# svg-project/Sparse-VideoGen

Hardware: AMD Instinct MI355X
Metric: attn_tflops_svg1_block_sparse (higher is better)
Workload: dtype bf16; 1 GPU; HunyuanVideo T2V hy720p SVG1 sparse layer-call: sample_mse(64 rows) + band attention with fused head placement, cfg=1 H=24 D=128 F=33 P=3600 ctx=256 prompt=64 S=119056 band=15616 density=0.2456; parallelism=single, variant=0, heads=alt

## Files before the change

### include/svg_attn.h

```cpp
#ifndef SVG_ATTN_H_
#define SVG_ATTN_H_

#include <stddef.h>
#include <stdint.h>

#ifdef __cplusplus
extern "C" {
#endif

#define SVG_DTYPE_BF16 0
#define SVG_DTYPE_F16 1
#define SVG_DTYPE_F32 2

#define SVG_OK 0
#define SVG_ERR_BAD_ARG (-1)
#define SVG_ERR_UNSUPPORTED (-2)
#define SVG_ERR_WORKSPACE (-3)
#define SVG_ERR_LAUNCH (-4)

#define SVG_ABI_VERSION 4
int svg_abi_version(void);

const char* svg_strerror(int code);
int svg_last_hip_error(void);
// ... 221 lines not shown
                           void* workspace, size_t workspace_bytes, const int32_t* skip_flag, void* stream);

size_t svg_band_attention_fp8_workspace_bytes(int32_t BH, int32_t S, int32_t D);
int svg_band_attention_fp8(const void* q, const void* k, const void* v, void* o, int32_t BH, int32_t S, int32_t D, int32_t dtype,
                           float sm_scale, const svg_band_mask_t* mask, const svg_perm_desc_t* perm, void* workspace,
                           size_t workspace_bytes, void* stream);
int svg_band_attention_fp8_stage(const void* q, const void* k, const void* v, void* o, int32_t BH, int32_t S, int32_t D, int32_t dtype,
                                 float sm_scale, const svg_band_mask_t* mask, const svg_perm_desc_t* perm, void* workspace,
                                 size_t workspace_bytes, int32_t stage, void* stream);

size_t svg_varblock_attention_fp8_workspace_bytes(int32_t Hq, int32_t Hkv, int32_t QB, int32_t KB, int32_t Sq, int32_t Skv, int32_t D);
int svg_varblock_attention_fp8(const void* q, const void* k, const void* v, void* o, int32_t Hq, int32_t Hkv, int32_t Sq, int32_t Skv,
                               int32_t D, int32_t dtype, float sm_scale, const uint8_t* block_map, const int32_t* q_sizes,
                               const int32_t* k_sizes, int32_t QB, int32_t KB, const int32_t* q_row_idx, const int32_t* kv_row_idx,
                               void* workspace, size_t workspace_bytes, void* stream);

int32_t svg_band_attention_notify_target(int32_t S, const svg_band_mask_t* mask);
int svg_band_attention_notify(const void* q, const void* k, const void* v, void* o, int32_t BH, int32_t S, int32_t D,
                              int32_t dtype, float sm_scale, const svg_band_mask_t* mask, const svg_perm_desc_t* perm,
                              int32_t* done_per_head, int32_t done_words, void* stream);
int svg_wait_counters(const int32_t* counters, int32_t n, int32_t target, void* stream);
int svg_wait_counters_deadline(const int32_t* counters, int32_t n, int32_t target, int32_t timeout_ms, int32_t* timed_out,
                               void* stream);
int32_t svg_band_attention_notify_layout(int32_t S, const svg_band_mask_t* mask, int32_t nseg, int32_t* row_bounds, int32_t* targets);
int svg_band_attention_notify_seg(const void* q, const void* k, const void* v, void* o, int32_t BH, int32_t S, int32_t D,
                                  int32_t dtype, float sm_scale, const svg_band_mask_t* mask, const svg_perm_desc_t* perm,
                                  int32_t* done, int32_t done_words, int32_t nseg, void* stream);
int svg_band_attention_prescaled_notify_seg(const void* q_scaled, const void* k, const void* v, void* o, int32_t BH, int32_t S,
                                            int32_t D, int32_t dtype, const svg_band_mask_t* mask, const svg_perm_desc_t* perm,
                                            int32_t* done, int32_t done_words, int32_t nseg, void* stream);

int32_t svg_band_queue_order(int32_t BH, int32_t S, const svg_band_mask_t* mask, int32_t* out, int32_t out_words);
int svg_debug_band_queue_cap(int32_t max_workgroups);

int svg_debug_pp_trace(uint64_t* out104);

int svg_debug_clock_probe(const int32_t* stop_flag, uint64_t* out2, int32_t max_ms, void* stream);

int svg_debug_wg_trace(uint64_t* out, int32_t n_workgroups);

#ifdef __cplusplus
}
#endif
#endif
```

### sparse-videogen_amd/csrc/attention.hip

```cpp
#include <algorithm>
#include <atomic>
#include <mutex>

#include "attn_core.h"
#include "attn_m16.h"
#include "band_policy.h"

namespace svg {

template <typename T, int D, int NW>
__global__ __launch_bounds__(NW * 64, 2) void band_attn_kernel(typename BandPolicy<T, D, NW>::Params prm) {
    extern __shared__ __attribute__((aligned(16))) char smem[];
    attn_body<T, D, NW, BandPolicy<T, D, NW>>(prm, smem, nullptr);
}

template <typename T, int D>
__global__ __launch_bounds__(512, (D == 64 ? 4 : 2)) void band_attn_pp2_kernel(typename BandPolicy<T, D, 8>::Params prm) {
    extern __shared__ __attribute__((aligned(16))) char smem[];
    attn_body_pp2<T, D, BandPolicy<T, D, 8>, false, 0, false, D == 64>(prm, smem, nullptr);
}
template <typename T>
__global__ __launch_bounds__(512, 4) void band_attn_pp2_switch64_kernel(typename BandPolicy<T, 64, 8>::Params prm,
                                                                        typename BandPolicy<T, 64, 8>::Params prm_alt,
                                                                        const int32_t* __restrict__ flag) {
    extern __shared__ __attribute__((aligned(16))) char smem[];
    if (flag[0] != 0) attn_body_pp2<T, 64, BandPolicy<T, 64, 8>, false, 0, false, true>(prm_alt, smem, nullptr);
    else attn_body_pp2<T, 64, BandPolicy<T, 64, 8>, false, 0, false, true>(prm, smem, nullptr);
}
template <typename T, int D>
__global__ __launch_bounds__(512, 2) void band_attn_pp2q_switch_kernel(typename BandPolicy<T, D, 8>::Params prm,
                                                                       typename BandPolicy<T, D, 8>::Params prm_alt,
                                                                       const int32_t* __restrict__ flag) {
    extern __shared__ __attribute__((aligned(16))) char smem[];
    if (flag[0] != 0) attn_body_pp2<T, D, BandPolicy<T, D, 8>, false, 0, true>(prm_alt, smem, nullptr);
    else attn_body_pp2<T, D, BandPolicy<T, D, 8>, false, 0, true>(prm, smem, nullptr);
}

__global__ __launch_bounds__(512, 2) void band_attn_pp2_frozen_kernel(typename BandPolicy<__bf16, 128, 8>::Params prm) {
    extern __shared__ __attribute__((aligned(16))) char smem[];
    attn_body_pp2<__bf16, 128, BandPolicy<__bf16, 128, 8>, false, 8>(prm, smem, nullptr);
}
template <typename T>
__global__ __launch_bounds__(512, 2) void band_attn_m16_kernel(typename BandPolicy<T, 128, 8>::Params prm) {
    extern __shared__ __attribute__((aligned(16))) char smem[];
    attn_body_m16<T, BandPolicy<T, 128, 8>, false, 1>(prm, smem, nullptr);
}
template <typename T>
__global__ __launch_bounds__(512, 2) void band_attn_m16q_kernel(typename BandPolicy<T, 128, 8>::Params prm) {
    extern __shared__ __attribute__((aligned(16))) char smem[];
    attn_body_m16<T, BandPolicy<T, 128, 8>, false, 1, true>(prm, smem, nullptr);
}
template <typename T, bool PRE = false>
__global__ __launch_bounds__(512, 2) void band_attn_m16_queue_kernel(typename BandPolicy<T, 128, 8>::Params prm, BandQueue qd) {
    extern __shared__ __attribute__((aligned(16))) char smem[];
    using Pol = BandPolicy<T, 128, 8>;
    int* const slot = (int*)(smem + attn_m16_lds_bytes());
    int dry = 0;
    for (;;) {
        if (threadIdx.x == 0) {
            const int xcd = __builtin_amdgcn_s_getreg((31 << 11) | 20) & (kNumXCD - 1);
            int head = -1, qt = 0;
            const int w = qd.take(xcd, dry);
            if (w >= 0) qd.decode(w, head, qt);
            slot[0] = head, slot[1] = qt;
        }
        __syncthreads();
        const int head = __builtin_amdgcn_readfirstlane(slot[0]), qt = __builtin_amdgcn_readfirstlane(slot[1]);
        if (head < 0) break;
        typename Pol::Ctx ctx;
        Pol::init_tile(prm, ctx, head, qt);
        attn_m16_tile<T, Pol, false, 1, PRE>(prm, ctx, smem);
    }
    if (threadIdx.x == 0) qd.leave(gridDim.x);
}
constexpr int kQueueLds = 16;
template <typename T, bool PRE = false>
__global__ __launch_bounds__(512, 2) void band_attn_m16_switch_kernel(typename BandPolicy<T, 128, 8>::Params prm,
                                                                      typename BandPolicy<T, 128, 8>::Params prm_alt,
                                                                      const int32_t* __restrict__ flag) {
    extern __shared__ __attribute__((aligned(16))) char smem[];
    if (flag[0] != 0) attn_body_m16<T, BandPolicy<T, 128, 8>, false, 1, PRE>(prm_alt, smem, nullptr);
    else attn_body_m16<T, BandPolicy<T, 128, 8>, false, 1, PRE>(prm, smem, nullptr);
}
template <typename T, int D>
__global__ __launch_bounds__(512, 2) void band_attn_pp2q_kernel(typename BandPolicy<T, D, 8>::Params prm) {
    extern __shared__ __attribute__((aligned(16))) char smem[];
    attn_body_pp2<T, D, BandPolicy<T, D, 8>, false, 0, true>(prm, smem, nullptr);
}
#ifdef SVG_ABLATIONS
template <typename T, int D, int ABL>
__global__ __launch_bounds__(512, 2) void band_attn_pp2_trace_kernel(typename BandPolicy<T, D, 8>::Params prm) {
    extern __shared__ __attribute__((aligned(16))) char smem[];
    attn_body_pp2<T, D, BandPolicy<T, D, 8>, true, ABL>(prm, smem, nullptr);
}
template <typename T>
__global__ __launch_bounds__(512, 2) void band_attn_m16_trace_kernel(typename BandPolicy<T, 128, 8>::Params prm) {
    extern __shared__ __attribute__((aligned(16))) char smem[];
    attn_body_m16<T, BandPolicy<T, 128, 8>, true>(prm, smem, nullptr);
}
template <typename T, int D>
__global__ __launch_bounds__(512, 2) void band_attn_pp2q_trace_kernel(typename BandPolicy<T, D, 8>::Params prm) {
    extern __shared__ __attribute__((aligned(16))) char smem[];
    attn_body_pp2<T, D, BandPolicy<T, D, 8>, true, 0, true>(prm, smem, nullptr);
}
#endif

int (*g_trace_reader)(uint64_t*, bool, int) = read_trace_here;

enum BandSchedule : int { kBandAuto = 0, kBandLockstep4 = 1, kBandPingPong = 2, kBandW4 = 3, kBandFrozen = 6, kBandM16 = 8 };
static inline int band_default(int D) { return D == 128 ? kBandM16 : kBandPingPong; }

int band_waves_per_tile(int variant) {
    const int v = variant == kBandAuto ? kBandPingPong : variant;
    return v == kBandW4 ? 4 : ((v == kBandPingPong || v == kBandM16) ? 8 : -1);
}
// ... 97 lines not shown
    if ((variant & 0xFF) == 32) {
        opts.trace = true;
        opts.trace_abl = (variant >> 8) & 15;
        return run_band_w4(q, k, v, o, BH, S, D, dtype, sm_scale, mask, perm, opts, st);
    }
    if (variant & 64) {
        trace_abl = (variant >> 8) & 15;
        variant = kBandPingPong;
        g_trace_reader = read_trace_here;
    }
    if (variant == kBandAuto) variant = band_default(D);
    if (opts.done && band_waves_per_tile(variant) < 0) return SVG_ERR_UNSUPPORTED;
    if (opts.strided && variant != kBandM16 && variant != kBandPingPong) return SVG_ERR_UNSUPPORTED;
    if (variant == kBandW4) return run_band_w4(q, k, v, o, BH, S, D, dtype, sm_scale, mask, perm, opts, st);
    if (variant != kBandLockstep4 && variant != kBandPingPong && variant != kBandFrozen && variant != kBandM16) return SVG_ERR_BAD_ARG;
    return dispatch_td(dtype, D, [&](auto t, auto d) -> int {
        using T = decltype(t);
        constexpr int DD = decltype(d)::value;
        using Pol = BandPolicy<T, DD, 8>;
        auto launch = [&](auto kern, int lds) {
            const typename Pol::Params p = make_band_params<Pol, T>(q, k, v, o, BH, S, sm_scale, mask, perm, opts);
            return launch_attn(kern, dim3(p.nqt * BH), 512, lds, st, p);
        };
        auto launch_queue = [&](auto kern_q, auto kern, int lds) {
            const typename Pol::Params p = make_band_params<Pol, T>(q, k, v, o, BH, S, sm_scale, mask, perm, opts);
            int n_cu = 0;
            int32_t* const block = opts.done ? nullptr : band_queue_block(st, n_cu);
            const int cap = band_queue_cap();
            if (!block || (p.nqt * BH <= n_cu && cap == 0)) return launch_attn(kern, dim3(p.nqt * BH), 512, lds, st, p);
            BandQueue qd = make_band_queue<Pol>(p);
            qd.ctr = block;
            int n_wg = std::min(qd.n_items, n_cu);
            if (cap > 0) n_wg = std::min(n_wg, cap);
            return launch_attn(kern_q, dim3(n_wg), 512, lds + kQueueLds, st, p, qd);
        };
        auto launch_switch = [&](auto kern, int lds) {
            const typename Pol::Params a = make_band_params<Pol, T>(q, k, v, o, BH, S, sm_scale, mask, perm, opts);
            const typename Pol::Params b = make_band_params<Pol, T>(q, k, v, o, BH, S, sm_scale, opts.alt_mask, nullptr, opts);
            return launch_attn(kern, dim3(std::max(a.nqt, b.nqt) * BH), 512, lds, st, a, b, opts.use_alt);
        };
        switch (variant) {
            case kBandLockstep4: {
                using Pol4 = BandPolicy<T, DD, 4>;
                const typename Pol4::Params p = make_band_params<Pol4, T>(q, k, v, o, BH, S, sm_scale, mask, perm, opts);
                return launch_attn(band_attn_kernel<T, DD, 4>, dim3(p.nqt * BH), 256, attn_lds_bytes<DD, 4>(), st, p);
            }
            case kBandPingPong:
#ifdef SVG_ABLATIONS
                if constexpr (DD == 128 && std::is_same<T, __bf16>::value) {
                    switch (trace_abl) {
#define SVG_PP_TRACE(A) case A: return launch(band_attn_pp2_trace_kernel<T, DD, A>, attn_pp2_lds_bytes<DD>());
                        SVG_PP_TRACE(0) SVG_PP_TRACE(1) SVG_PP_TRACE(2) SVG_PP_TRACE(4) SVG_PP_TRACE(5) SVG_PP_TRACE(6) SVG_PP_TRACE(7) SVG_PP_TRACE(8)
#undef SVG_PP_TRACE
                        case -1: break;
                        case 3: return launch(band_attn_pp2q_trace_kernel<T, DD>, attn_pp2_lds_bytes<DD>());
                        case 9: return launch(band_attn_m16_trace_kernel<T>, attn_m16_lds_bytes());
                        default: return SVG_ERR_UNSUPPORTED;
                    }
                }
#endif
                if (trace_abl >= 0) return SVG_ERR_UNSUPPORTED;
                if (opts.use_alt) {
                    if (opts.prescaled) return launch_switch(band_attn_pp2q_switch_kernel<T, DD>, attn_pp2_lds_bytes<DD>());
                    if constexpr (DD == 64) return launch_switch(band_attn_pp2_switch64_kernel<T>, attn_pp2_lds_bytes<64>());
                    return SVG_ERR_UNSUPPORTED;
                }
                return launch(opts.prescaled ? band_attn_pp2q_kernel<T, DD> : band_attn_pp2_kernel<T, DD>, attn_pp2_lds_bytes<DD>());
            case kBandFrozen:
                if constexpr (DD == 128 && std::is_same<T, __bf16>::value) {
                    if (opts.done || opts.prescaled) return SVG_ERR_UNSUPPORTED;
                    return launch(band_attn_pp2_frozen_kernel, attn_pp2_lds_bytes<128>());
                }
                return SVG_ERR_UNSUPPORTED;
            default:
                if constexpr (DD == 128) {
                    if (opts.use_alt)
                        return launch_switch(opts.prescaled ? band_attn_m16_switch_kernel<T, true> : band_attn_m16_switch_kernel<T>,
                                             attn_m16_lds_bytes());
                    if (opts.prescaled) return launch_queue(band_attn_m16_queue_kernel<T, true>, band_attn_m16q_kernel<T>, attn_m16_lds_bytes());
                    return launch_queue(band_attn_m16_queue_kernel<T>, band_attn_m16_kernel<T>, attn_m16_lds_bytes());
                }
                return SVG_ERR_UNSUPPORTED;
        }
    });
}

extern "C" int svg_band_attention(const void* q, const void* k, const void* v, void* o, int32_t BH, int32_t S, int32_t D,
                                  int32_t dtype, float sm_scale, const svg_band_mask_t* mask,
                                  const svg_perm_desc_t* perm, int32_t variant, void* stream) {
    return band_dispatch(q, k, v, o, BH, S, D, dtype, sm_scale, mask, perm, variant, BandOpts(), 0, nullptr, stream);
}

extern "C" int svg_band_attention_strided(const void* q, const void* k, const void* v, void* o, int32_t BH, int32_t S, int32_t D,
                                          int32_t dtype, float sm_scale, const svg_band_mask_t* mask, const svg_perm_desc_t* perm,
                                          const svg_attn_layout_t* layout, void* stream) {
    BandOpts opts;
    opts.strided = true;
    return band_dispatch(q, k, v, o, BH, S, D, dtype, sm_scale, mask, perm, kBandAuto, opts, 0, layout, stream);
}

extern "C" int svg_band_attention_prescaled(const void* q_scaled, const void* k, const void* v, void* o, int32_t BH, int32_t S,
                                            int32_t D, int32_t dtype, const svg_band_mask_t* mask, const svg_perm_desc_t* perm,
                                            void* stream) {
    BandOpts opts;
    opts.prescaled = true;
    return band_dispatch(q_scaled, k, v, o, BH, S, D, dtype, 1.f, mask, perm, kBandAuto, opts, 0, nullptr, stream);
}

extern "C" int32_t svg_band_attention_notify_target(int32_t S, const svg_band_mask_t* mask) {
    if (!mask || S <= 0) return -1;
    using Pol = svg::BandPolicy<__bf16, 128, 8>;
    const auto p = svg::make_band_params<Pol, __bf16>(nullptr, nullptr, nullptr, nullptr, 1, S, 1.f, mask, nullptr);
    return p.nqt * band_waves_per_tile(kBandAuto);
// ... 93 lines not shown
    BandOpts opts = switch_opts(alt_mask, use_alt_flag);
    opts.prescaled = true;
    return band_dispatch(q_scaled, k, v, o, BH, S, D, dtype, 1.f, mask, perm, kBandAuto, opts, 0, nullptr, stream);
}

extern "C" int32_t svg_band_queue_order(int32_t BH, int32_t S, const svg_band_mask_t* mask, int32_t* out, int32_t out_words) {
    if (!mask || BH <= 0 || S <= 0 || check_band_mask(S, mask, nullptr) != SVG_OK) return -1;
    using Pol = svg::BandPolicy<__bf16, 128, 8>;
    const auto p = svg::make_band_params<Pol, __bf16>(nullptr, nullptr, nullptr, nullptr, BH, S, 1.f, mask, nullptr);
    const BandQueue qd = svg::make_band_queue<Pol>(p);
    if (!out) return qd.n_items;
    int n = 0;
    for (int x = 0; x <= kNumXCD; ++x)
        for (unsigned i = 0;; ++i) {
            const int w = x < kNumXCD ? qd.item(x, i) : qd.tail_item(i);
            if (w < 0) break;
            if (3 * (n + 1) > out_words) return -1;
            int head, qt;
            qd.decode(w, head, qt);
            Pol::Ctx c;
            Pol::kv_schedule(p, c, qt);
            out[3 * n] = x, out[3 * n + 1] = head * p.nqt + qt, out[3 * n + 2] = c.nT;
            ++n;
        }
    return n;
}

extern "C" int svg_debug_band_queue_cap(int32_t max_workgroups) {
    if (max_workgroups < 0) return SVG_ERR_BAD_ARG;
    g_queue_cap.store(max_workgroups, std::memory_order_relaxed);
    return SVG_OK;
}

extern "C" int svg_debug_wg_trace(uint64_t* out, int n_workgroups) { return g_trace_reader(out, true, n_workgroups); }
extern "C" int svg_debug_pp_trace(uint64_t* out104) { return g_trace_reader(out104, false, 0); }
```

### sparse-videogen_amd/csrc/attn_m16.h

```cpp
#pragma once
#include "attn_core.h"

namespace svg {

template <typename T>
struct Mfma16;
template <>
struct Mfma16<__bf16> {
    static __device__ __forceinline__ f32x4 mfma(bf16x8 a, bf16x8 b, f32x4 c) { return __builtin_amdgcn_mfma_f32_16x16x32_bf16(a, b, c, 0, 0, 0); }
    static __device__ __forceinline__ f32x4 mfma_keep_c(bf16x8 a, bf16x8 b, const f32x4& c) {
        f32x4 d;
        asm volatile("v_mfma_f32_16x16x32_bf16 %0, %1, %2, %3" : "=&v"(d) : "v"(a), "v"(b), "v"(c));
        return d;
    }
};
template <>
struct Mfma16<_Float16> {
    static __device__ __forceinline__ f32x4 mfma(f16x8 a, f16x8 b, f32x4 c) { return __builtin_amdgcn_mfma_f32_16x16x32_f16(a, b, c, 0, 0, 0); }
    static __device__ __forceinline__ f32x4 mfma_keep_c(f16x8 a, f16x8 b, const f32x4& c) {
        f32x4 d;
        asm volatile("v_mfma_f32_16x16x32_f16 %0, %1, %2, %3" : "=&v"(d) : "v"(a), "v"(b), "v"(c));
        return d;
    }
};

constexpr int attn_m16_lds_bytes() { return attn_pp2_lds_bytes<128>(); }

__device__ __forceinline__ float quad_group_max(float x) {
    x = vmax2(x, __shfl_xor(x, 16));
    return vmax2(x, __shfl_xor(x, 32));
}
__device__ __forceinline__ float quad_group_sum(float x) {
    x += __shfl_xor(x, 16);
    return x + __shfl_xor(x, 32);
}

template <typename T, typename P, bool TRACE = false, int ONEBAR = -1, bool PRE = false>
__device__ __forceinline__ void attn_m16_tile(const typename P::Params& prm, const typename P::Ctx& ctx, char* smem) {
    using E = Elt<T>;
    using M = Mfma16<T>;
    using V8 = typename E::v8;
    constexpr int D = 128;
    constexpr int NW = 8;
    constexpr int KS = D / 32;
    constexpr int NDB = D / 16;
    constexpr int NS = 4;
    constexpr int kImg = kBN * D * 2;
    constexpr int kStage = 2 * kImg;
    constexpr int NP = 2;
    constexpr int kCarry = 8;
    constexpr int kPF = 8;
    constexpr bool kOneBar = ONEBAR < 0 ? P::kOneBarrier : (ONEBAR != 0);
    static_assert(P::kRowBlocks == 1 && !P::kPartialOut && !P::kFixup && P::kIntervalMask, "band / variable-block policy");
    constexpr bool MSUM = std::is_same_v<T, __bf16> && !PRE;
    constexpr float kBias = MSUM ? 10.f : 0.f;

    unsigned long long wg_t0 = 0, wg_t2 = 0;
    if constexpr (TRACE) wg_t0 = __builtin_amdgcn_s_memtime();
    const int tid = threadIdx.x;
    const int lane = tid & 63;
    const int wave = wave_id();
    const int g4 = lane >> 4;
    const int n16 = lane & 15;
    const bool lagging = wave >= NW / 2;
    const int nT = ctx.nT;

    const T* __restrict__ qb = P::q_base(prm, ctx);
    const T* __restrict__ kb_ = P::k_base(prm, ctx);
    const T* __restrict__ vb = P::v_base(prm, ctx);
    const unsigned lds0 = (unsigned)(size_t)smem;

    const int dma_kg = wave / 2;
    const int dma_db0 = (wave % 2) * NP;
    const int krow = 16 * dma_kg + (lane >> 2);
    typename P::KvCursor cur;
    P::kv_cursor_init(prm, ctx, cur, krow);
    const unsigned vsw = (unsigned)((lane >> 4) & 1) << 1;
    const unsigned col_v = (unsigned)(dma_db0 * 64 + (((lane & 3) ^ vsw) * 16));
    const unsigned lds_piece = lds0 + (unsigned)(dma_db0 * (kBN * 64) + dma_kg * 1024);
    int nphys = 0, nnext = 0;
    auto resolve = [&](int t, auto guard_c) {
        if constexpr (decltype(guard_c)::value) nnext = (t < nT) ? P::kv_phys(prm, ctx, cur, t, krow) : 0;
        else nnext = P::kv_phys(prm, ctx, cur, t, krow);
    };
    constexpr std::true_type kGuarded{};
    auto take = [&]() { nphys = nnext; };
    const unsigned k_rsb = (unsigned)P::k_rs(prm) * 2u, v_rsb = (unsigned)P::v_rs(prm) * 2u;
    auto dma_piece = [&](int t, auto j_c) {
        constexpr int j = decltype(j_c)::value;
        const unsigned st = __builtin_amdgcn_readfirstlane(lds_piece + (unsigned)((t % NS) * kStage) + j * (kBN * 64));
        const unsigned ko = __umul24((unsigned)nphys, k_rsb) + col_v;
        const unsigned vo = __umul24((unsigned)nphys, v_rsb) + col_v;
        const char* const kbp = (const char*)kb_ + j * 64;
        const char* const vbp = (const char*)vb + j * 64;
        asm volatile("s_mov_b32 m0, %0\n\t"
                     "s_nop 0\n\t"
                     "global_load_lds_dwordx4 %1, %3\n\t"
                     "s_add_u32 m0, m0, %5\n\t"
// ... 11 lines not shown
    for (int t = 0; t < dist; ++t) {
        resolve(t, kGuarded);
        take();
        if (t < nT) dma_issue(t);
    }
    resolve(dist, kGuarded);

    int q_log[2];
    V8 qf[2][KS];
    int m_a0[2], m_b0[2];
    unsigned m_alen[2], m_blen[2];
#pragma unroll
    for (int rb = 0; rb < 2; ++rb) {
        const int row_in_wg = wave * 32 + rb * 16 + n16;
        const int qp = P::q_phys(prm, ctx, row_in_wg);
        q_log[rb] = P::q_logical(ctx, row_in_wg);
        const T* qrow = qb + (size_t)(qp >= 0 ? qp : 0) * P::q_rs(prm) + g4 * 8;
#pragma unroll
        for (int ks = 0; ks < KS; ++ks) qf[rb][ks] = *(const V8*)(qrow + ks * 32);
        P::row_intervals(prm, ctx, q_log[rb], m_a0[rb], m_alen[rb], m_b0[rb], m_blen[rb]);
    }

    const int k_lane = n16 * 64 + ((g4 ^ (((n16 >> 2) & 1) << 1)) << 4);
    const int v_lane0 = kImg + (4 * g4 + (n16 >> 2)) * 64 + (((g4 & 1) * 16) + 4 * (n16 & 3)) * 2;
    const int v_lane1 = v_lane0 ^ 32;

    float m_run[2] = {-INFINITY, -INFINITY}, m_use[2] = {0.f, 0.f}, l_run[2] = {0.f, 0.f}, psum[2] = {0.f, 0.f};
    float m_sub[2] = {kBias, kBias};
    f32x4 acc_l[2] = {{0.f, 0.f, 0.f, 0.f}, {0.f, 0.f, 0.f, 0.f}};
    V8 ones8;
#pragma unroll
    for (int j = 0; j < 8; ++j) ones8[j] = E::from_float(1.f);
    bool force_exact = true;
    f32x4 acc_o[NDB][2];
#pragma unroll
    for (int db = 0; db < NDB; ++db)
#pragma unroll
        for (int rb = 0; rb < 2; ++rb)
#pragma unroll
            for (int r = 0; r < 4; ++r) acc_o[db][rb][r] = 0.f;
    const float c_log2 = prm.scale_log2;
    if constexpr (MSUM) asm volatile("" : "+v"(ones8));

#pragma unroll
    for (int rb = 0; rb < 2; ++rb)
#pragma unroll
        for (int ks = 0; ks < KS; ++ks) asm volatile("" : "+v"(qf[rb][ks]));
    asm volatile("s_waitcnt vmcnt(0)" ::: "memory");
    pp_barrier();
    if (!kOneBar && lagging) pp_barrier();

    const bool idle = !P::wave_active(ctx, wave * 32);

    unsigned tr_acc[4] = {0, 0, 0, 0};
    unsigned long long tr_last = 0, tr_first = 0;
    if constexpr (TRACE) tr_first = tr_last = __builtin_amdgcn_s_memtime();
    auto tick = [&](auto slot_c) {
        if constexpr (TRACE) {
            constexpr int slot = decltype(slot_c)::value;
            const unsigned long long now = __builtin_amdgcn_s_memtime();
            tr_acc[slot] += (unsigned)(now - tr_last);
            tr_last = now;
        }
    };

    f32x4 neg_ref[2] = {{0.f, 0.f, 0.f, 0.f}, {0.f, 0.f, 0.f, 0.f}};
// ... 44 lines not shown
        if (more) dma_piece(t + dist, std::integral_constant<int, 0>{});
        const int tk0 = P::tile_key0(ctx, t);
        const int cls = P::classify(prm, ctx, tk0, wave * 32);
        if (cls != TILE_FULL) {
            const bool part = (cls == TILE_PARTIAL);
#pragma unroll
            for (int rb = 0; rb < 2; ++rb) {
                int ka = tk0 + 4 * g4 - m_a0[rb], kb2 = tk0 + 4 * g4 - m_b0[rb];
                asm volatile("" : "+v"(ka), "+v"(kb2));
#pragma unroll
                for (int b = 0; b < 4; ++b)
#pragma unroll
                    for (int r = 0; r < 4; ++r) {
                        const int key = 16 * b + r;
                        const bool ok = ((unsigned)(ka + key) < m_alen[rb]) | ((unsigned)(kb2 + key) < m_blen[rb]);
                        sc[b][rb][r] = (part & ok) ? sc[b][rb][r] : -INFINITY;
                    }
            }
        }
        if (more) dma_piece(t + dist, std::integral_constant<int, 1>{});
        psum[0] = 0.f, psum[1] = 0.f;
#pragma unroll
        for (int kc = 0; kc < 2; ++kc) {
            probs(kc);
            asm volatile("" : "+v"(pf[kc][0]), "+v"(pf[kc][1]), "+v"(psum[0]), "+v"(psum[1]));
        }
        bool exact;
        if constexpr (MSUM) {
            typedef unsigned u32x4_t __attribute__((ext_vector_type(4)));
            const u32x4_t w0 = __builtin_bit_cast(u32x4_t, pf[0][0]), w1 = __builtin_bit_cast(u32x4_t, pf[0][1]);
            const u32x4_t w2 = __builtin_bit_cast(u32x4_t, pf[1][0]), w3 = __builtin_bit_cast(u32x4_t, pf[1][1]);
            const unsigned o0 = w0[0] | w0[1] | w0[2], o1 = w0[3] | w1[0] | w1[1], o2 = w1[2] | w1[3] | w2[0];
            const unsigned o3 = w2[1] | w2[2] | w2[3], o4 = w3[0] | w3[1] | w3[2];
            const unsigned bits = (o0 | o1 | o2) | (o3 | o4 | w3[3]);
            exact = force_exact || __any((bits & 0x40004000u) != 0u);
        } else {
            exact = !__all(psum[0] + psum[1] <= psum_thr);
        }
        if (exact) {
            bool all_finite = true;
            float alpha[2];
#pragma unroll
            for (int rb = 0; rb < 2; ++rb) {
                float mx = vmax3(sc[0][rb][0], sc[0][rb][1], sc[0][rb][2]);
                mx = vmax3(mx, sc[0][rb][3], sc[1][rb][0]);
                mx = vmax3(mx, sc[1][rb][1], sc[1][rb][2]);
                mx = vmax3(mx, sc[1][rb][3], sc[2][rb][0]);
                mx = vmax3(mx, sc[2][rb][1], sc[2][rb][2]);
                mx = vmax3(mx, sc[2][rb][3], sc[3][rb][0]);
                mx = vmax3(mx, sc[3][rb][1], sc[3][rb][2]);
                mx = vmax2(mx, sc[3][rb][3]);
                const float m_prev = m_use[rb];
                mx = quad_group_max(mx);
                if constexpr (PRE) mx += m_prev;
                else mx *= c_log2;
                const float m_new = fmaxf(m_run[rb], mx);
                m_use[rb] = (m_new == -INFINITY) ? m_prev : m_new;
                m_sub[rb] = m_use[rb] + kBias;
                float a = __builtin_amdgcn_exp2f(fminf(m_prev - m_use[rb], 126.f));
                asm volatile("s_nop 1" : "+v"(a));
                alpha[rb] = a;
                m_run[rb] = m_new;
                all_finite = all_finite && (m_new != -INFINITY);
                l_run[rb] *= a;
                if constexpr (MSUM) {
#pragma unroll
                    for (int r = 0; r < 4; ++r) {
                        float x = acc_l[rb][r];
                        asm volatile("v_mul_f32 %0, %1, %0" : "+v"(x) : "v"(a));
                        acc_l[rb][r] = x;
                    }
                }
                if constexpr (PRE) {
                    pre_shift[rb] = m_prev - m_use[rb];
                    const float nm = -m_use[rb];
#pragma unroll
                    for (int r = 0; r < 4; ++r) {
                        float c = neg_ref[rb][r];
                        asm volatile("v_mov_b32 %0, %1" : "+v"(c) : "v"(nm));
                        neg_ref[rb][r] = c;
                    }
                }
            }
            psum_thr = __all(all_finite) ? 2048.f : -1.f;
            force_exact = !__all(all_finite);
#pragma unroll
            for (int db = 0; db < NDB; ++db)
#pragma unroll
                for (int rb = 0; rb < 2; ++rb)
#pragma unroll
                    for (int r = 0; r < 4; ++r) {
                        float x = acc_o[db][rb][r];
                        asm volatile("v_mul_f32 %0, %1, %0" : "+v"(x) : "v"(alpha[rb]));
                        acc_o[db][rb][r] = x;
                    }
            psum[0] = 0.f, psum[1] = 0.f;
#pragma unroll
            for (int kc = 0; kc < 2; ++kc) {
                probs_impl(kc, std::true_type{});
                asm volatile("" : "+v"(pf[kc][0]), "+v"(pf[kc][1]), "+v"(psum[0]), "+v"(psum[1]));
            }
        }
        if (more) asm volatile("s_waitcnt vmcnt(%0)" ::"n"(2 * NP) : "memory");
        else asm volatile("s_waitcnt vmcnt(0)" ::: "memory");
    };
    constexpr int NPV = 2 * NDB;
    constexpr int kMsumAt = 0;
    i16x8 ring[kPF + 1];
    i16x8 carry[kCarry];
    auto carry_load = [&](int t, int i) { carry[i] = vfrag(smem + (t % NS) * kStage, i / NDB, i % NDB); };
    auto matrix_phase = [&](int t, auto has_next_c) {
        constexpr bool has_next = decltype(has_next_c)::value;
        constexpr int NALL = has_next ? NPV + 4 * KS : NPV;
        const char* stv = smem + (t % NS) * kStage;
        const char* stk = smem + ((t + 1) % NS) * kStage;
        const f32x4 zero = {0.f, 0.f, 0.f, 0.f};
        auto fetch = [&](int i) {
            if (i >= NALL) return;
// ... 15 lines not shown
            }
            if (i < NPV) {
                const int kc = i / NDB, db = i % NDB;
                const V8 a = __builtin_bit_cast(V8, i < kCarry ? carry[i < kCarry ? i : 0] : ring[i % (kPF + 1)]);
                acc_o[db][0] = M::mfma(a, pf[kc][0], acc_o[db][0]);
                acc_o[db][1] = M::mfma(a, pf[kc][1], acc_o[db][1]);
                if constexpr (MSUM) {
                    if (db == kMsumAt) {
                        acc_l[0] = M::mfma(ones8, pf[kc][0], acc_l[0]);
                        acc_l[1] = M::mfma(ones8, pf[kc][1], acc_l[1]);
                    }
                } else {
                    if (i == NPV - 1) l_run[0] += psum[0], l_run[1] += psum[1];
                }
            } else {
                const int j = i - NPV, ks = j >> 2, b = j & 3;
                const V8 a = __builtin_bit_cast(V8, ring[i % (kPF + 1)]);
                if constexpr (PRE) {
                    sc[b][0] = ks == 0 ? M::mfma_keep_c(a, qf[0][ks], neg_ref[0]) : M::mfma(a, qf[0][ks], sc[b][0]);
                    sc[b][1] = ks == 0 ? M::mfma_keep_c(a, qf[1][ks], neg_ref[1]) : M::mfma(a, qf[1][ks], sc[b][1]);
                } else {
                    sc[b][0] = M::mfma(a, qf[0][ks], ks == 0 ? zero : sc[b][0]);
                    sc[b][1] = M::mfma(a, qf[1][ks], ks == 0 ? zero : sc[b][1]);
                }
            }
            __builtin_amdgcn_sched_barrier(0);
        }
        if constexpr (has_next) {
#pragma unroll
            for (int b = 0; b < 4; ++b) asm volatile("" : "+v"(sc[b][0]), "+v"(sc[b][1]));
        }
    };

    if (idle) {
        for (int t = 0; t < nT; ++t) {
            if (!kOneBar || lagging) pp_barrier();
            stage_resolve_next(t, kGuarded);
            stage_request(t);
            if (!kOneBar || !lagging) pp_barrier();
        }
        pp_barrier();
        if (!kOneBar && !lagging) pp_barrier();
        P::notify(prm, ctx);
        return;
    }

    if (nT > 0) {
        const f32x4 zero = {0.f, 0.f, 0.f, 0.f};
#pragma unroll
        for (int ks = 0; ks < KS; ++ks)
#pragma unroll
            for (int b = 0; b < 4; ++b) {
                const V8 a = __builtin_bit_cast(V8, kfrag(smem, b, ks));
                sc[b][0] = M::mfma(a, qf[0][ks], ks == 0 ? zero : sc[b][0]);
                sc[b][1] = M::mfma(a, qf[1][ks], ks == 0 ? zero : sc[b][1]);
            }
#pragma unroll
        for (int b = 0; b < 4; ++b) asm volatile("" : "+v"(sc[b][0]), "+v"(sc[b][1]));
#pragma unroll
        for (int i = 0; i < kCarry; ++i) carry_load(0, i);
    }
    const int bar_n = lagging ? 1 : 0, bar_m = lagging ? 0 : 1;
    auto tile = [&](int t, auto has_next_c, auto guard_c) {
        tick(std::integral_constant<int, 0>{});
        if constexpr (kOneBar) pp_barrier_if(bar_n);
        else pp_barrier();
        tick(std::integral_constant<int, 1>{});
        vector_phase(t, guard_c);
        tick(std::integral_constant<int, 2>{});
        if constexpr (kOneBar) pp_barrier_if(bar_m);
        else pp_barrier();
        tick(std::integral_constant<int, 3>{});
        __builtin_amdgcn_s_setprio(1);
        matrix_phase(t, has_next_c);
        __builtin_amdgcn_s_setprio(0);
    };
    int t = 0;
    for (const int n_main = nT - dist - 1; t < n_main; ++t) tile(t, std::true_type{}, std::false_type{});
    for (; t + 1 < nT; ++t) tile(t, std::true_type{}, kGuarded);
    if (nT > 0) tile(nT - 1, std::false_type{}, kGuarded);
    pp_barrier();
    if (!kOneBar && !lagging) pp_barrier();
    if constexpr (TRACE) {
        if (blockIdx.x == kPpTraceBlock && lane == 0) {
#pragma unroll
            for (int j = 0; j < 4; ++j) g_pp_trace[wave * 8 + j] = tr_acc[j];
            if (wave == 0) g_pp_trace[64] = (unsigned long long)nT, g_pp_trace[65] = tr_last - tr_first;
        }
        wg_t2 = __builtin_amdgcn_s_memtime();
    }

    constexpr int kEpiStride = D * 2 + 8;
    char* erow = smem + (size_t)(wave * 32) * kEpiStride;
#pragma unroll
    for (int rb = 0; rb < 2; ++rb) {
        const float l_tot = MSUM ? acc_l[rb][0] : quad_group_sum(l_run[rb]);
        const float inv = l_tot > 0.f ? 1.f / l_tot : 0.f;
#pragma unroll
        for (int db = 0; db < NDB; ++db) {
            typename E::v4 o4;
#pragma unroll
            for (int j = 0; j < 4; ++j) o4[j] = E::from_float(acc_o[db][rb][j] * inv);
            *(typename E::v4*)(erow + (rb * 16 + n16) * kEpiStride + (16 * db + 4 * g4) * 2) = o4;
        }
    }
    __builtin_amdgcn_s_waitcnt(0xc07f);
    __builtin_amdgcn_wave_barrier();
    T* __restrict__ ob = P::o_base(prm, ctx);
    const int o_rs = P::o_rs(prm);
    constexpr int kLanesPerRow = D * 2 / 8;
    constexpr int kRowsPerPass = 64 / kLanesPerRow;
    const int sub = lane / kLanesPerRow;
    const int colb = (lane - sub * kLanesPerRow) * 8;
    int ephys[32 / kRowsPerPass];
#pragma unroll
    for (int i = 0; i < 32 / kRowsPerPass; ++i) ephys[i] = P::q_phys(prm, ctx, wave * 32 + i * kRowsPerPass + sub);
#pragma unroll
    for (int i = 0; i < 32 / kRowsPerPass; ++i) {
        const int rr = i * kRowsPerPass + sub;
        const u32x2 val = *(const u32x2*)(erow + rr * kEpiStride + colb);
        if (ephys[i] >= 0) *(u32x2*)((char*)(ob + (size_t)ephys[i] * o_rs) + colb) = val;
    }
    P::notify(prm, ctx);
    if constexpr (TRACE) {
        asm volatile("s_waitcnt vmcnt(0)" ::: "memory");
        if (wave == 0 && lane == 0 && blockIdx.x < (unsigned)kWgTraceMax) {
            unsigned long long* w = g_wg_trace + (size_t)blockIdx.x * 6;
            w[0] = wg_t0, w[1] = tr_first, w[2] = wg_t2, w[3] = __builtin_amdgcn_s_memtime();
            w[4] = __builtin_amdgcn_s_getreg((31 << 11) | 4);
            w[5] = __builtin_amdgcn_s_getreg((31 << 11) | 20);
        }
    }
}

template <typename T, typename P, bool TRACE = false, int ONEBAR = -1, bool PRE = false>
__device__ __forceinline__ void attn_body_m16(const typename P::Params& prm, char* smem, char* policy_lds) {
    typename P::Ctx ctx;
    if (!P::init(prm, ctx, policy_lds)) return;
    attn_m16_tile<T, P, TRACE, ONEBAR, PRE>(prm, ctx, smem);
}

}
```

### sparse-videogen_amd/svg/_native.py

```python
from __future__ import annotations

import ctypes as C
import os
from pathlib import Path
from typing import NamedTuple, Optional, Sequence

import torch

_LIB_PATH = Path(__file__).resolve().parent.parent / "lib" / "libsvgattn.so"
_lib: Optional[C.CDLL] = None
_load_error: Optional[str] = None

SVG_DTYPE_BF16, SVG_DTYPE_F16 = 0, 1


class BandMask(C.Structure):

    _fields_ = [
        ("real_len", C.c_int32),
        ("band", C.c_int32),
        ("colfull_lo", C.c_int32),
        ("colfull_hi", C.c_int32),
        ("rowfull_lo", C.c_int32),
        ("rowfull_hi", C.c_int32),
# ... 33 lines not shown
        ("num_frame", C.c_int32),
        ("frame_size", C.c_int32),
        ("emulate_bf16", C.c_int32),
        ("variant", ProfileVariant * 2),
    ]


_I32, _I64, _F32, _VP, _SZ = C.c_int32, C.c_int64, C.c_float, C.c_void_p, C.c_size_t


class PrologueSegment(C.Structure):
    _fields_ = [("q_in", C.c_void_p), ("k_in", C.c_void_p), ("v_in", C.c_void_p), ("rows", C.c_int32), ("norm_kind", C.c_int32),
                ("q_weight", C.c_void_p), ("q_bias", C.c_void_p), ("k_weight", C.c_void_p), ("k_bias", C.c_void_p), ("eps", C.c_float)]


class TensorStrides(C.Structure):
    _fields_ = [("batch", C.c_int64), ("head", C.c_int64), ("row", C.c_int64)]


class AttnLayout(C.Structure):
    _fields_ = [("heads_per_batch", C.c_int32), ("kv_heads_per_batch", C.c_int32), ("q", TensorStrides), ("k", TensorStrides),
                ("v", TensorStrides), ("o", TensorStrides)]


SIGNATURES = {
    "svg_abi_version": (C.c_int, []),
    "svg_strerror": (C.c_char_p, [C.c_int]),
    "svg_last_hip_error": (C.c_int, []),
    "svg_build_info": (C.c_char_p, []),
    "svg_debug_pp_trace": (C.c_int, [_VP]),
    "svg_debug_wg_trace": (C.c_int, [_VP, _I32]),
    "svg_band_queue_order": (_I32, [_I32, _I32, C.POINTER(BandMask), _VP, _I32]),
    "svg_debug_band_queue_cap": (C.c_int, [_I32]),
    "svg_rms_norm_forward": (C.c_int, [_VP, _VP, C.c_int64, _I32, _I32, C.c_float, _VP]),
    "svg_layer_norm_forward": (C.c_int, [_VP, _VP, _VP, C.c_int64, _I32, _I32, _VP]),
    "svg_apply_qk_rope_inplace_cossin": (C.c_int, [_VP, _VP, _VP, _VP, _I32, _I32, _I32, _I32, _I32, _I32, _I32, _VP]),
    "svg_apply_qk_rope_inplace_cossin_txtlast": (C.c_int, [_VP, _VP, _VP, _VP, _I32, _I32, _I32, _I32, _I32, _I32, _I32, _VP]),
    "svg_apply_qk_rope_inplace_cossin_complex": (C.c_int, [_VP, _VP, _VP, _VP, _I32, _I32, _I32, _I32, _I32, _I32, _I32, _VP]),
    "svg_bsr_to_block_map": (C.c_int, [_VP, _VP, _I32, _I32, _I32, _I32, _I32, _I32, _VP, _VP, _VP, _VP]),
    "svg_layernorm_forward": (C.c_int, [_VP, _VP, _VP, _VP, C.c_int64, _I32, _I32, _I32, _I32, C.c_float, _VP]),
    "svg_rmsnorm_forward": (C.c_int, [_VP, _VP, _VP, C.c_int64, _I32, _I32, _I32, _I32, C.c_float, _VP]),
    "svg_layernorm_forward_ex": (C.c_int, [_VP, _VP, _VP, _VP, C.c_int64, _I32, _I32, _I32, _I32, C.c_float, _I32, _VP]),
    "svg_modulate_shift_forward": (C.c_int, [_VP, _VP, _VP, _VP, C.c_int64, _I32, C.c_int64, _I32, _I32, _VP]),
    "svg_modulate_gate_residual_forward": (C.c_int, [_VP, _VP, _VP, _VP, C.c_int64, _I32, C.c_int64, _I32, _I32, _I32, _VP]),
    "svg_layernorm_modulate_forward": (C.c_int, [_VP, _VP, _VP, _VP, _VP, _VP, C.c_int64, _I32, C.c_int64, _I32, _I32, _I32,
                                                 C.c_float, _VP]),
    "svg_layernorm_modulate_forward_ex": (C.c_int, [_VP, _VP, _VP, _VP, _VP, _VP, C.c_int64, _I32, C.c_int64, _I32, _I32, _I32,
                                                    C.c_float, _I32, _VP]),
    "svg_qk_norm_rope_transpose": (C.c_int, [_VP, _VP, _VP, _VP, _I32, _I32, _I32, _I32, _I32, _I32, _I32, _VP, _VP, _VP, _VP,
                                             C.c_float, _I32, _VP, _VP, _I32, _I32, _VP]),
    "svg_qk_norm_rope": (C.c_int, [_VP, _VP, _I32, _I32, _I32, _I32, _I32, _I32, _I32, _VP, _VP, _VP, _VP, C.c_float, _I32, _VP,
                                   _VP, _I32, _I32, _VP]),
    "svg_qk_norm_rope_qscale": (C.c_int, [_VP, _VP, _I32, _I32, _I32, _I32, _I32, _I32, _I32, _VP, _VP, _VP, _VP, C.c_float, _I32, _VP,
                                          _VP, _I32, _I32, C.c_float, _VP]),
    "svg_qk_norm_rope_transpose_qscale": (C.c_int, [_VP, _VP, _VP, _VP, _I32, _I32, _I32, _I32, _I32, _I32, _I32, _VP, _VP, _VP, _VP,
                                                    C.c_float, _I32, _VP, _VP, _I32, _I32, C.c_float, _VP]),
    "svg_qk_norm_rope_transpose_joint": (C.c_int, [C.POINTER(PrologueSegment), _I32, _VP, _VP, _VP, _I32, _I32, _I32, _I32, _I32, _VP, _VP,
                                                   _I32, _I32, C.c_float, _VP]),
    "svg_rmsnorm_rope_transpose": (C.c_int, [_VP, _VP, _VP, _VP, _VP, _VP, _I32, _I32, _I32, _I32, _I32, _VP, _VP, _I32, C.c_float, _I32, _VP,
                                             _VP, _I32, _I32, C.c_float, _VP]),
    "svg_head_placement": (C.c_int, [_VP, _VP, _I32, _VP, _I32, _I32, _I32, _I32, _I32, _I32, _I32, _I32, _I32, _VP]),
    "svg_permute_rows": (C.c_int, [_VP, _VP, _VP, _I32, _I32, _I32, _I32, _VP]),
    "svg_inverse_permute_rows": (C.c_int, [_VP, _VP, _VP, _I32, _I32, _I32, _I32, _VP]),
    "svg_argsort_workspace_bytes": (_SZ, [_I32, _I32, _I32]),
    "svg_argsort_labels": (C.c_int, [_VP, _VP, _VP, _I32, _I32, _I32, _VP, _SZ, _VP]),
    "svg_band_attention": (C.c_int, [_VP, _VP, _VP, _VP, _I32, _I32, _I32, _I32, _F32, C.POINTER(BandMask),
# ... 359 lines not shown
    o = torch.empty_like(q) if out is None else out
    _dev(o)
    scale = _sm_scale(sm_scale, D)
    perm = _perm_arg(head_perm_flag, BH, vid0, num_frame, frame_size)
    need = int(lib.svg_band_attention_fp8_workspace_bytes(BH, S, D))
    if need == 0:
        raise RuntimeError(f"svg_band_attention_fp8: unsupported shape (D = {D}; only 128)")
    if workspace is None:
        key = WorkspaceCache.key("band", BH, S, device=q.device)
        workspace = _F8_WS.get(key)
        if workspace is None or workspace.numel() < need:
            workspace = _F8_WS[key] = torch.empty(need, dtype=torch.uint8, device=q.device)
    _dev(workspace)
    assert workspace.dtype == torch.uint8 and workspace.numel() >= need
    args = (q.data_ptr(), k.data_ptr(), v.data_ptr(), o.data_ptr(), BH, S, D, _dtype_code(q), scale, C.byref(mask), perm,
            workspace.data_ptr(), workspace.numel())
    if stage:
        _check(lib.svg_band_attention_fp8_stage(*args, int(stage), _stream()), "svg_band_attention_fp8_stage")
    else:
        _check(lib.svg_band_attention_fp8(*args, _stream()), "svg_band_attention_fp8")
    return o


def notify_counters(BH: int, nseg: int, device) -> torch.Tensor:
    return torch.zeros(BH * (nseg + 1), device=device, dtype=torch.int32)


def band_notify_target(S: int, mask: BandMask) -> int:
    t = load().svg_band_attention_notify_target(int(S), C.byref(mask))
    assert t > 0
    return int(t)


def band_notify_layout(S: int, mask: BandMask, nseg: int):
    rb = (C.c_int32 * (nseg + 1))()
    tg = (C.c_int32 * nseg)()
    n = load().svg_band_attention_notify_layout(int(S), C.byref(mask), int(nseg), C.cast(rb, C.c_void_p), C.cast(tg, C.c_void_p))
    assert n > 0
    return n, list(rb)[: n + 1], list(tg)[:n]


def wait_counters(counters: torch.Tensor, target: int, timeout_ms: int = 0, timed_out: Optional[torch.Tensor] = None) -> None:
    _dev(counters)
    assert counters.dtype == torch.int32 and counters.is_contiguous()
    if timeout_ms > 0:
        assert timed_out is not None, "wait_counters(timeout_ms > 0) needs a `timed_out` flag tensor (int32 [1] on the GPU)"
        _dev(timed_out)
        assert timed_out.dtype == torch.int32 and timed_out.numel() >= 1
        _check(load().svg_wait_counters_deadline(counters.data_ptr(), counters.numel(), int(target), int(timeout_ms),
                                                 timed_out.data_ptr(), _stream()), "svg_wait_counters_deadline")
        return
    _check(load().svg_wait_counters(counters.data_ptr(), counters.numel(), int(target), _stream()), "svg_wait_counters")


def band_attention_switch(q: torch.Tensor, k: torch.Tensor, v: torch.Tensor, mask: BandMask, alt_mask: BandMask,
                          use_alt_flag: torch.Tensor, sm_scale: Optional[float] = None,
                          head_perm_flag: Optional[torch.Tensor] = None, vid0: int = 0, num_frame: int = 1, frame_size: int = 1,
                          out: Optional[torch.Tensor] = None, q_prescaled: bool = False, token_major_out: bool = False) -> torch.Tensor:
    _dev(use_alt_flag)
    assert use_alt_flag.dtype == torch.int32 and use_alt_flag.numel() >= 1
    return _band_attention(q, k, v, mask, alt_mask, use_alt_flag, sm_scale, head_perm_flag, vid0, num_frame, frame_size, 0, out, None, 1,
                           q_prescaled, token_major_out)


def cross_attention_supported(q: torch.Tensor, k: torch.Tensor) -> bool:
    return (q.is_cuda and k.is_cuda and q.dtype in (torch.bfloat16, torch.float16) and k.dtype == q.dtype
# ... 617 lines not shown
```

Measured before the change: 1313 TFLOP/s.

## Speculatively skip per-tile exactness check in bf16 m16 band attention, replay on overflow

In the bf16 m16 band attention kernels, the per-tile 'exact' overflow check on scores now runs only every kCheckEvery tiles once the running max is finite. At the end of the tile the accumulators are validated, and if any are non-finite or too large the whole tile is replayed with full checking, coordinated through an LDS flag. This cuts per-iteration check and vote overhead in the inner loop, at the cost of an extra barrier at tile end, extra LDS, and occasional full recomputation. A debug counter for replays is exposed.

```diff
diff --git a/include/svg_attn.h b/include/svg_attn.h
--- a/include/svg_attn.h
+++ b/include/svg_attn.h
@@ -277,6 +277,7 @@
 
 int32_t svg_band_queue_order(int32_t BH, int32_t S, const svg_band_mask_t* mask, int32_t* out, int32_t out_words);
 int svg_debug_band_queue_cap(int32_t max_workgroups);
+int64_t svg_debug_band_replays(int32_t reset);
 
 int svg_debug_pp_trace(uint64_t* out104);
 
diff --git a/sparse-videogen_amd/csrc/attention.hip b/sparse-videogen_amd/csrc/attention.hip
--- a/sparse-videogen_amd/csrc/attention.hip
+++ b/sparse-videogen_amd/csrc/attention.hip
@@ -40,10 +40,12 @@
     extern __shared__ __attribute__((aligned(16))) char smem[];
     attn_body_pp2<__bf16, 128, BandPolicy<__bf16, 128, 8>, false, 8>(prm, smem, nullptr);
 }
+static __device__ unsigned g_band_replays;
+constexpr int kTailLds = 16;
 template <typename T>
 __global__ __launch_bounds__(512, 2) void band_attn_m16_kernel(typename BandPolicy<T, 128, 8>::Params prm) {
     extern __shared__ __attribute__((aligned(16))) char smem[];
-    attn_body_m16<T, BandPolicy<T, 128, 8>, false, 1>(prm, smem, nullptr);
+    attn_body_m16<T, BandPolicy<T, 128, 8>, false, 1, false, true>(prm, smem, nullptr, &g_band_replays);
 }
 template <typename T>
 __global__ __launch_bounds__(512, 2) void band_attn_m16q_kernel(typename BandPolicy<T, 128, 8>::Params prm) {
@@ -55,32 +57,47 @@
     extern __shared__ __attribute__((aligned(16))) char smem[];
     using Pol = BandPolicy<T, 128, 8>;
     int* const slot = (int*)(smem + attn_m16_lds_bytes());
+    constexpr bool kSpec = !PRE && std::is_same_v<T, __bf16>;
     int dry = 0;
+    if constexpr (kSpec) {
+        if (threadIdx.x == 0) slot[2] = 0;
+    }
     for (;;) {
         if (threadIdx.x == 0) {
-            const int xcd = __builtin_amdgcn_s_getreg((31 << 11) | 20) & (kNumXCD - 1);
-            int head = -1, qt = 0;
-            const int w = qd.take(xcd, dry);
-            if (w >= 0) qd.decode(w, head, qt);
-            slot[0] = head, slot[1] = qt;
+            bool fresh = true;
+            if constexpr (kSpec) {
+                fresh = __builtin_amdgcn_readfirstlane(slot[2]) != 1;
+                slot[2] = fresh ? 0 : 2;
+            }
+            if (fresh) {
+                const int xcd = __builtin_amdgcn_s_getreg((31 << 11) | 20) & (kNumXCD - 1);
+                int head = -1, qt = 0;
+                const int w = qd.take(xcd, dry);
+                if (w >= 0) qd.decode(w, head, qt);
+                slot[0] = head, slot[1] = qt;
+            }
         }
         __syncthreads();
         const int head = __builtin_amdgcn_readfirstlane(slot[0]), qt = __builtin_amdgcn_readfirstlane(slot[1]);
         if (head < 0) break;
         typename Pol::Ctx ctx;
         Pol::init_tile(prm, ctx, head, qt);
-        attn_m16_tile<T, Pol, false, 1, PRE>(prm, ctx, smem);
+        if constexpr (kSpec) {
+            const int check_mask = __builtin_amdgcn_readfirstlane(slot[2]) == 2 ? 0 : kCheckEvery - 1;
+            attn_m16_tile<T, Pol, false, 1, PRE, true>(prm, ctx, smem, check_mask, &g_band_replays);
+        } else {
+            attn_m16_tile<T, Pol, false, 1, PRE>(prm, ctx, smem);
+        }
     }
     if (threadIdx.x == 0) qd.leave(gridDim.x);
 }
-constexpr int kQueueLds = 16;
 template <typename T, bool PRE = false>
 __global__ __launch_bounds__(512, 2) void band_attn_m16_switch_kernel(typename BandPolicy<T, 128, 8>::Params prm,
                                                                       typename BandPolicy<T, 128, 8>::Params prm_alt,
                                                                       const int32_t* __restrict__ flag) {
     extern __shared__ __attribute__((aligned(16))) char smem[];
-    if (flag[0] != 0) attn_body_m16<T, BandPolicy<T, 128, 8>, false, 1, PRE>(prm_alt, smem, nullptr);
-    else attn_body_m16<T, BandPolicy<T, 128, 8>, false, 1, PRE>(prm, smem, nullptr);
+    if (flag[0] != 0) attn_body_m16<T, BandPolicy<T, 128, 8>, false, 1, PRE, !PRE>(prm_alt, smem, nullptr, &g_band_replays);
+    else attn_body_m16<T, BandPolicy<T, 128, 8>, false, 1, PRE, !PRE>(prm, smem, nullptr, &g_band_replays);
 }
 template <typename T, int D>
 __global__ __launch_bounds__(512, 2) void band_attn_pp2q_kernel(typename BandPolicy<T, D, 8>::Params prm) {
@@ -244,7 +261,7 @@
             qd.ctr = block;
             int n_wg = std::min(qd.n_items, n_cu);
             if (cap > 0) n_wg = std::min(n_wg, cap);
-            return launch_attn(kern_q, dim3(n_wg), 512, lds + kQueueLds, st, p, qd);
+            return launch_attn(kern_q, dim3(n_wg), 512, lds, st, p, qd);
         };
         auto launch_switch = [&](auto kern, int lds) {
             const typename Pol::Params a = make_band_params<Pol, T>(q, k, v, o, BH, S, sm_scale, mask, perm, opts);
@@ -288,9 +305,10 @@
                 if constexpr (DD == 128) {
                     if (opts.use_alt)
                         return launch_switch(opts.prescaled ? band_attn_m16_switch_kernel<T, true> : band_attn_m16_switch_kernel<T>,
-                                             attn_m16_lds_bytes());
-                    if (opts.prescaled) return launch_queue(band_attn_m16_queue_kernel<T, true>, band_attn_m16q_kernel<T>, attn_m16_lds_bytes());
-                    return launch_queue(band_attn_m16_queue_kernel<T>, band_attn_m16_kernel<T>, attn_m16_lds_bytes());
+                                             attn_m16_lds_bytes() + kTailLds);
+                    if (opts.prescaled)
+                        return launch_queue(band_attn_m16_queue_kernel<T, true>, band_attn_m16q_kernel<T>, attn_m16_lds_bytes() + kTailLds);
+                    return launch_queue(band_attn_m16_queue_kernel<T>, band_attn_m16_kernel<T>, attn_m16_lds_bytes() + kTailLds);
                 }
                 return SVG_ERR_UNSUPPORTED;
         }
@@ -450,5 +468,13 @@
     return SVG_OK;
 }
 
+extern "C" int64_t svg_debug_band_replays(int32_t reset) {
+    unsigned n = 0;
+    if (hipDeviceSynchronize() != hipSuccess || hipMemcpyFromSymbol(&n, HIP_SYMBOL(g_band_replays), sizeof n) != hipSuccess) return -1;
+    const unsigned zero = 0;
+    if (reset && hipMemcpyToSymbol(HIP_SYMBOL(g_band_replays), &zero, sizeof zero) != hipSuccess) return -1;
+    return (int64_t)n;
+}
+
 extern "C" int svg_debug_wg_trace(uint64_t* out, int n_workgroups) { return g_trace_reader(out, true, n_workgroups); }
 extern "C" int svg_debug_pp_trace(uint64_t* out104) { return g_trace_reader(out104, false, 0); }
diff --git a/sparse-videogen_amd/csrc/attn_m16.h b/sparse-videogen_amd/csrc/attn_m16.h
--- a/sparse-videogen_amd/csrc/attn_m16.h
+++ b/sparse-videogen_amd/csrc/attn_m16.h
@@ -35,8 +35,10 @@
     return x + __shfl_xor(x, 32);
 }
 
-template <typename T, typename P, bool TRACE = false, int ONEBAR = -1, bool PRE = false>
-__device__ __forceinline__ void attn_m16_tile(const typename P::Params& prm, const typename P::Ctx& ctx, char* smem) {
+constexpr int kCheckEvery = 8;
+template <typename T, typename P, bool TRACE = false, int ONEBAR = -1, bool PRE = false, bool SPEC = false>
+__device__ __forceinline__ bool attn_m16_tile(const typename P::Params& prm, const typename P::Ctx& ctx, char* smem,
+                                              int check_mask = kCheckEvery - 1, unsigned* replay_ctr = nullptr) {
     using E = Elt<T>;
     using M = Mfma16<T>;
     using V8 = typename E::v8;
@@ -54,6 +56,8 @@
     static_assert(P::kRowBlocks == 1 && !P::kPartialOut && !P::kFixup && P::kIntervalMask, "band / variable-block policy");
     constexpr bool MSUM = std::is_same_v<T, __bf16> && !PRE;
     constexpr float kBias = MSUM ? 10.f : 0.f;
+    constexpr bool kSpec = SPEC && MSUM;
+    static_assert(!(SPEC && TRACE) && (kCheckEvery & (kCheckEvery - 1)) == 0, "SPEC: product kernels; a power of two");
 
     unsigned long long wg_t0 = 0, wg_t2 = 0;
     if constexpr (TRACE) wg_t0 = __builtin_amdgcn_s_memtime();
@@ -64,6 +68,7 @@
     const int n16 = lane & 15;
     const bool lagging = wave >= NW / 2;
     const int nT = ctx.nT;
+    volatile int* const spec_word = (volatile int*)(smem + attn_m16_lds_bytes() + 8);
 
     const T* __restrict__ qb = P::q_base(prm, ctx);
     const T* __restrict__ kb_ = P::k_base(prm, ctx);
@@ -141,6 +146,7 @@
 #pragma unroll
     for (int j = 0; j < 8; ++j) ones8[j] = E::from_float(1.f);
     bool force_exact = true;
+    int spec_mode = -1;
     f32x4 acc_o[NDB][2];
 #pragma unroll
     for (int db = 0; db < NDB; ++db)
@@ -251,8 +257,16 @@
             const u32x4_t w2 = __builtin_bit_cast(u32x4_t, pf[1][0]), w3 = __builtin_bit_cast(u32x4_t, pf[1][1]);
             const unsigned o0 = w0[0] | w0[1] | w0[2], o1 = w0[3] | w1[0] | w1[1], o2 = w1[2] | w1[3] | w2[0];
             const unsigned o3 = w2[1] | w2[2] | w2[3], o4 = w3[0] | w3[1] | w3[2];
-            const unsigned bits = (o0 | o1 | o2) | (o3 | o4 | w3[3]);
-            exact = force_exact || __any((bits & 0x40004000u) != 0u);
+            if constexpr (kSpec) {
+                exact = spec_mode < 0;
+                if (spec_mode >= 0 && (t & spec_mode) == 0) {
+                    const unsigned bits = (o0 | o1 | o2) | (o3 | o4 | w3[3]);
+                    exact = __builtin_amdgcn_readfirstlane((int)__any((bits & 0x40004000u) != 0u)) != 0;
+                }
+            } else {
+                const unsigned bits = (o0 | o1 | o2) | (o3 | o4 | w3[3]);
+                exact = force_exact || __any((bits & 0x40004000u) != 0u);
+            }
         } else {
             exact = !__all(psum[0] + psum[1] <= psum_thr);
         }
@@ -303,6 +317,7 @@
             }
             psum_thr = __all(all_finite) ? 2048.f : -1.f;
             force_exact = !__all(all_finite);
+            if constexpr (kSpec) spec_mode = force_exact ? -1 : check_mask;
 #pragma unroll
             for (int db = 0; db < NDB; ++db)
 #pragma unroll
@@ -384,6 +399,14 @@
         }
     };
 
+    auto spec_replay = [&](bool bad) -> bool {
+        if (__any(bad) && lane == 0) *spec_word = 1;
+        pp_barrier();
+        if (__builtin_amdgcn_readfirstlane(*spec_word) == 0) return false;
+        if (replay_ctr && tid == 0) atomicAdd(replay_ctr, 1u);
+        return true;
+    };
+
     if (idle) {
         for (int t = 0; t < nT; ++t) {
             if (!kOneBar || lagging) pp_barrier();
@@ -393,8 +416,11 @@
         }
         pp_barrier();
         if (!kOneBar && !lagging) pp_barrier();
+        if constexpr (kSpec) {
+            if (check_mask != 0 && spec_replay(false)) return true;
+        }
         P::notify(prm, ctx);
-        return;
+        return false;
     }
 
     if (nT > 0) {
@@ -441,6 +467,18 @@
         }
         wg_t2 = __builtin_amdgcn_s_memtime();
     }
+    if constexpr (kSpec) {
+        if (check_mask != 0) {
+            bool bad = !(fabsf(acc_l[0][0]) < 0x1p120f) || !(fabsf(acc_l[1][0]) < 0x1p120f);
+#pragma unroll
+            for (int db = 0; db < NDB; ++db)
+#pragma unroll
+                for (int rb = 0; rb < 2; ++rb)
+#pragma unroll
+                    for (int r = 0; r < 4; ++r) bad = bad || !(fabsf(acc_o[db][rb][r]) < 0x1p120f);
+            if (spec_replay(bad)) return true;
+        }
+    }
 
     constexpr int kEpiStride = D * 2 + 8;
     char* erow = smem + (size_t)(wave * 32) * kEpiStride;
@@ -483,13 +521,21 @@
             w[5] = __builtin_amdgcn_s_getreg((31 << 11) | 20);
         }
     }
+    return false;
 }
 
-template <typename T, typename P, bool TRACE = false, int ONEBAR = -1, bool PRE = false>
-__device__ __forceinline__ void attn_body_m16(const typename P::Params& prm, char* smem, char* policy_lds) {
+template <typename T, typename P, bool TRACE = false, int ONEBAR = -1, bool PRE = false, bool SPEC = false>
+__device__ __forceinline__ void attn_body_m16(const typename P::Params& prm, char* smem, char* policy_lds, unsigned* replay_ctr = nullptr) {
     typename P::Ctx ctx;
     if (!P::init(prm, ctx, policy_lds)) return;
-    attn_m16_tile<T, P, TRACE, ONEBAR, PRE>(prm, ctx, smem);
+    if constexpr (SPEC && std::is_same_v<T, __bf16> && !PRE) {
+        if (threadIdx.x == 0) *(volatile int*)(smem + attn_m16_lds_bytes() + 8) = 0;
+#pragma nounroll
+        for (int check_mask = kCheckEvery - 1;; check_mask = 0)
+            if (!attn_m16_tile<T, P, TRACE, ONEBAR, PRE, SPEC>(prm, ctx, smem, check_mask, replay_ctr)) break;
+    } else {
+        attn_m16_tile<T, P, TRACE, ONEBAR, PRE>(prm, ctx, smem);
+    }
 }
 
 }
diff --git a/sparse-videogen_amd/svg/_native.py b/sparse-videogen_amd/svg/_native.py
--- a/sparse-videogen_amd/svg/_native.py
+++ b/sparse-videogen_amd/svg/_native.py
@@ -89,6 +89,7 @@
     "svg_debug_wg_trace": (C.c_int, [_VP, _I32]),
     "svg_band_queue_order": (_I32, [_I32, _I32, C.POINTER(BandMask), _VP, _I32]),
     "svg_debug_band_queue_cap": (C.c_int, [_I32]),
+    "svg_debug_band_replays": (C.c_int64, [_I32]),
     "svg_rms_norm_forward": (C.c_int, [_VP, _VP, C.c_int64, _I32, _I32, C.c_float, _VP]),
     "svg_layer_norm_forward": (C.c_int, [_VP, _VP, _VP, C.c_int64, _I32, _I32, _VP]),
     "svg_apply_qk_rope_inplace_cossin": (C.c_int, [_VP, _VP, _VP, _VP, _I32, _I32, _I32, _I32, _I32, _I32, _I32, _VP]),
@@ -514,6 +515,13 @@
     return int(t)
 
 
+def band_replays(reset: bool = False) -> int:
+    n = int(load().svg_debug_band_replays(1 if reset else 0))
+    if n < 0:
+        raise RuntimeError("svg_debug_band_replays failed")
+    return n
+
+
 def band_notify_layout(S: int, mask: BandMask, nseg: int):
     rb = (C.c_int32 * (nseg + 1))()
     tg = (C.c_int32 * nseg)()
```

New measurement: 1334 TFLOP/s (median of 6 runs). 1.6% higher.
